# HpWang-whu/RoReg

Hardware: AMD Instinct MI355X
Metric: pair-registrations/sec (higher is better)
Workload: dtype f32 (every f32 operand enters the fp16 matrix cores as hi + lo fp16 under a per-keypoint power-of-two block scale: <= 22 significant bits relative to a CONSERVATIVE per-keypoint bound -- measured on the extractor: the bound sits 2^2..2^6 above the keypoint's true coefficient maximum (config.f16x2_sc

## Files before the change

include/roreg_hip.h:

```cpp
#ifndef ROREG_HIP_H
#define ROREG_HIP_H

#include <stdint.h>
#include <stddef.h>

#ifdef __cplusplus
extern "C" {
#endif

#define ROREG_ABI_VERSION 6
int roreg_abi_version(void);
const char *roreg_last_error(void);

int roreg_set_group_tables(const int32_t *P_host, const int32_t *Nei_host, const double *R_host);

size_t roreg_group_conv_packed_size(int Cin, int Cout, int KS);
int roreg_group_conv_pack_weights(const float *W_host , int Cin, int Cout, int KS,
                                  float *wpack_host );
size_t roreg_group_conv_workspace_size(int B, int Cin, int Cout, int Lin, int Lout, int KS);
int roreg_group_conv(const float *x, const float *wpack, const float *bias,
                     const float *bn_scale, const float *bn_shift, const float *residual,
                     float *out, const int32_t *gather,
                     int B, int Cin, int Cout, int Lin, int Lout, int KS,
                     float *workspace, size_t workspace_floats, void *stream);
// ... 215 lines not shown
size_t roreg_irrep_gemm_tiles(int O, int B, int32_t *tiles_host);
size_t roreg_irrep_gemm_tiles_m(int O, int B, int tile_m , int32_t *tiles_host);
int roreg_irrep_gemm(const float *const *X, float *const *Out, const float *const *Add, const float *const *Wpack, int C, int O, int B,
                     const int32_t *tiles_dev, int n_tiles, void *stream);
int roreg_irrep_gemm_split(const float *const *X, float *const *Out, const float *const *Add, const void *const *Wsplit, int C, int O, int B,
                           const int32_t *tiles_dev, int n_tiles, void *stream);
int roreg_irrep_gemm_f16x2(const float *const *X, float *const *Out, const float *const *Add, const void *const *Wsplit2,
                           const float *x_bound_dev, int w_exp, const float *next_u_dev, const float *next_v_dev, float *out_bound_dev,
                           int C, int O, int B, const int32_t *tiles_dev, int n_tiles,
                           int tile_m ,
                           int x_planes , void *stream);
int roreg_gemm_persistent(int on);
int roreg_gemm_thin(int on);
int roreg_irrep_gemm_f16x2_rows(const float *const *X, float *T3r, const void *const *Wsplit2, const float *x_bound_dev, int w_exp, int C, int B, void *stream);
int roreg_gf_finish(const float *T3r, const float *x, const float *b_out, const float *role_scale , const float *role_shift ,
                    float *eqv, float *inv, float *role_out , float *eqv_ft, int B, void *stream);
int roreg_gf_finish_route(int on);
int roreg_row_bound(const void *x_spatial, int x_bf16 , const float *bn_scale, const float *bn_shift,
                    float *bound_out, int B, int C, void *stream);
int roreg_ft_nonlin(const float *Xin , const float *x_spatial, const float *bias,
                    const float *bias2, const float *bn_scale, const float *bn_shift, const float *resid_spatial,
                    float *Xout , float *out_spatial ,
                    const int32_t *g_map ,
                    int Lout , int Lvalid,
                    int B, int C, int split ,
                    const float *out_bound ,
                    float *out_rowmax ,
                    int spatial_bf16 ,
                    int out_planes ,
                    void *stream);
int roreg_ft_nonlin_packed(const float *Xin, const float *bias, const float *bn_scale, const float *bn_shift, uint32_t *out_words,
                           const int32_t *g_map, int Lout, int Lvalid, int B, int C, const float *out_bound, float *raw_col, int raw_g,
                           void *stream);
int roreg_ft_nonlin_gathered(const uint64_t *rows , const int64_t *dr , int feat_bf16, const float *bn_scale ,
                             const float *bn_shift, float *Xout, int B, const float *out_bound , int out_planes, void *stream);

typedef struct roreg_icp_grid_desc {
    double origin[3];
    double edge;
    int32_t dims[3];
    int32_t n;
    int64_t cells;
    int64_t reserved;
} roreg_icp_grid_desc;
size_t roreg_icp_grid_size(const double *lo_host, const double *hi_host, int n, double max_dist, roreg_icp_grid_desc *desc_host,
                           size_t *workspace_bytes);
int roreg_icp_grid_build(const float *points, const roreg_icp_grid_desc *desc_host, void *grid, void *workspace, size_t workspace_bytes,
                         void *stream);
typedef struct roreg_icp_task {
    const void *tgt_grid;
    const void *src_grid;
    const double *T0;
    int32_t n_src;
    int32_t slot0;
} roreg_icp_task;
size_t roreg_icp_batch_workspace(int n_tasks, long long total_slots);
int roreg_icp_batch(const roreg_icp_task *tasks, int n_tasks, const int32_t *work, int n_work, long long total_slots, double max_dist,
                    int max_iter, double tol_deg, double tol_t, double *T_out, int32_t *iters_out, int32_t *inliers_out, double *rmse_out,
                    int32_t *status_out, int32_t *assign_out, double *stats_out, void *workspace, size_t workspace_bytes, void *stream);

int roreg_icp_normals(const void *grid, double radius, int min_neighbors, double *out, void *stream);
typedef struct roreg_icp_plane_task {
    const void *tgt_grid;
    const void *src_grid;
    const double *tgt_normals;
    const double *T0;
// ... 151 lines not shown
```

roreg_amd/_abi.py:

```python
import ctypes
from ctypes import c_int, c_void_p, c_size_t, c_double, c_float, c_char_p

import numpy as np

ABI_VERSION = 6

_P = c_void_p
PROTOTYPES = {
    'roreg_abi_version': (c_int, []),
    'roreg_last_error': (c_char_p, []),
    'roreg_set_group_tables': (c_int, [_P, _P, _P]),
    'roreg_group_conv_packed_size': (c_size_t, [c_int, c_int, c_int]),
    'roreg_group_conv_pack_weights': (c_int, [_P, c_int, c_int, c_int, _P]),
    'roreg_group_conv_workspace_size': (c_size_t, [c_int, c_int, c_int, c_int, c_int, c_int]),
    'roreg_group_conv': (c_int, [_P, _P, _P, _P, _P, _P, _P, _P, c_int, c_int, c_int, c_int, c_int, c_int, _P, c_size_t, _P]),
    'roreg_group_conv_split': (c_int, [_P, _P, _P, _P, _P, _P, _P, _P, c_int, c_int, c_int, c_int, c_int, c_int, c_int, _P]),
    'roreg_group_conv_f16x2': (c_int, [_P, _P, c_int, _P, _P, _P, c_float, c_float, _P, _P, _P, _P, _P, c_int, c_int, c_int, c_int, c_int, c_int, c_int, _P]),
    'roreg_group_conv_f16x2_packed': (c_int, [_P, _P, c_int, _P, _P, _P, _P, _P, _P, c_int, c_int, c_int, c_int, c_int, c_int, c_int, _P]),
    'roreg_dense_f16x2': (c_int, [_P, _P, c_int, _P, _P, _P, c_float, c_float, _P, _P, c_int, _P, _P, c_int, c_int, c_int, _P]),
    'roreg_dense_split': (c_int, [_P, _P, _P, _P, _P, _P, c_int, _P, c_int, c_int, c_int, _P]),
    'roreg_gf_finalize': (c_int, [_P, _P, c_int, _P, c_int, _P]),
    'roreg_det_score': (c_int, [_P, _P, c_int, _P]),
    'roreg_inv_descriptor': (c_int, [_P, c_int, _P, c_int, _P]),
    'roreg_nn_search': (c_int, [_P, _P, c_int, _P, _P, c_int, c_int, _P, _P, _P, _P]),
# ... 24 lines not shown
    'roreg_row_bound_roles': (c_int, [_P, c_int, _P, _P, _P, _P, c_int, _P]),
    'roreg_inv_descriptor_roles': (c_int, [_P, c_int, _P, _P, _P, _P, c_int, _P]),
    'roreg_lt_prepare_rows': (c_int, [_P, _P, c_int, c_int, c_int, _P, _P, _P, _P]),
    'roreg_ransac_batch_workspace': (c_size_t, [c_int, ctypes.c_longlong, c_int]),
    'roreg_ransac_batch': (c_int, [_P, c_int, ctypes.c_longlong, c_int, c_int, c_double, c_int, _P, _P, _P, _P, _P, _P, c_size_t, _P]),
    'roreg_refine_batch': (c_int, [_P, _P, c_int, ctypes.c_longlong, _P, ctypes.c_double, c_int, _P, _P, _P, _P]),
    'roreg_yohoc_draw': (c_int, [_P, ctypes.c_longlong, _P, _P, c_int, c_int, _P, _P, _P, _P]),
    'roreg_gather_rows_batch': (c_int, [_P, c_int, c_int, c_int, _P]),
    'roreg_gather_rows_f64': (c_int, [_P, _P, c_int, c_int, _P, _P]),
    'roreg_group_corr': (c_int, [_P, _P, _P, _P, c_int, c_int, _P, _P, _P]),
    'roreg_topk_dot_workspace_size': (c_size_t, [c_int, c_int, c_int]),
    'roreg_topk_dot': (c_int, [_P, c_int, _P, c_int, c_int, _P, _P, _P, c_size_t, _P, _P, c_int, c_int, c_int, _P]),
    'roreg_context_colmax': (c_int, [_P, c_int, _P, c_int, c_int, _P, _P, _P]),
    'roreg_sinkhorn_batch_workspace_size': (c_size_t, [c_int, c_int, c_int, ctypes.c_longlong, ctypes.c_longlong]),
    'roreg_sinkhorn_batch_consts': (c_int, [_P, _P, c_int, _P]),
    'roreg_sinkhorn_batch': (c_int, [_P, _P, _P, _P, _P, _P, _P, c_int, c_float, c_int, _P, _P, _P, _P, _P, c_size_t, _P]),
    'roreg_sinkhorn_batch2_workspace_size': (c_size_t, [c_int, c_int, c_int, ctypes.c_longlong, ctypes.c_longlong]),
    'roreg_sinkhorn_batch2': (c_int, [_P, _P, _P, _P, _P, _P, _P, c_int, c_float, c_int, _P, _P, _P, _P, _P, c_size_t, c_int, _P]),
    'roreg_sinkhorn_batch3_workspace_size': (c_size_t, [c_int, c_int, c_int, ctypes.c_longlong, ctypes.c_longlong, c_int, c_int]),
    'roreg_sinkhorn_batch3': (c_int, [_P, _P, _P, _P, _P, _P, _P, c_int, c_float, c_int, _P, _P, _P, _P, _P, c_size_t, c_int, _P, _P]),
    'roreg_write_files': (c_int, [_P, _P, _P, _P, _P, c_int, c_int]),
    'roreg_yohoc_draw_many': (c_int, [_P, c_int, _P, _P, c_int, c_int, _P, _P, _P, c_int]),
    'roreg_mlp_head_workspace': (c_size_t, [c_int, c_int, c_int]),
    'roreg_mlp_head': (c_int, [_P, _P, _P, _P, _P, c_int, c_int, c_int, c_int, _P, _P, c_int, _P, _P, _P, _P, _P, c_int, c_int, c_float, _P, _P, _P]),
    'roreg_sinkhorn_early_exit': (c_int, [c_int]),
    'roreg_sinkhorn_iteration_stats': (c_int, [_P, _P, c_int, _P]),
    'roreg_linear': (c_int, [_P, c_int, c_int, _P, _P, c_int, _P, _P]),
    'roreg_linear_mfma': (c_int, [_P, c_int, c_int, _P, _P, c_int, _P, _P]),
    'roreg_linear_path': (c_int, [c_int]),
    'roreg_linear_cat3': (c_int, [_P, _P, _P, _P, c_int, c_int, _P, _P, c_int, _P, _P]),
    'roreg_gemm_persistent': (c_int, [c_int]),
    'roreg_gemm_thin': (c_int, [c_int]),
    'roreg_gf_finish_route': (c_int, [c_int]),
    'roreg_irrep_gemm_f16x2_rows': (c_int, [_P, _P, _P, _P, c_int, c_int, c_int, _P]),
    'roreg_gf_finish': (c_int, [_P, _P, _P, _P, _P, _P, _P, _P, _P, c_int, _P]),
    'roreg_instnorm_stats': (c_int, [_P, c_int, c_int, c_float, _P, _P, _P, c_int, c_int, _P]),
    'roreg_mlp_tail': (c_int, [_P, c_int, c_int, _P, _P, _P, _P, _P, c_int, c_int, _P]),
    'roreg_mlp_tail_mfma': (c_int, [_P, c_int, c_int, _P, _P, _P, _P, _P, c_int, c_int, _P]),
    'roreg_knn_attention': (c_int, [_P, _P, _P, _P, c_int, c_int, c_int, c_int, _P, _P]),
    'roreg_rm_elementwise': (c_int, [c_int, _P, _P, _P, _P, c_int, c_int, c_int, _P, _P, _P]),
    'roreg_sinkhorn_workspace_size': (c_size_t, [c_int, c_int]),
    'roreg_sinkhorn': (c_int, [_P, c_int, _P, c_int, c_float, c_int, _P, _P, _P, _P, _P, _P, c_size_t, _P]),
    'roreg_icp_grid_size': (c_size_t, [_P, _P, c_int, c_double, _P, _P]),
    'roreg_icp_grid_build': (c_int, [_P, _P, _P, _P, c_size_t, _P]),
    'roreg_icp_batch_workspace': (c_size_t, [c_int, ctypes.c_longlong]),
    'roreg_icp_batch': (c_int, [_P, c_int, _P, c_int, ctypes.c_longlong, c_double, c_int, c_double, c_double, _P, _P, _P, _P, _P, _P, _P, _P, c_size_t, _P]),
    'roreg_icp_normals': (c_int, [_P, c_double, c_int, _P, _P]),
    'roreg_icp_plane_batch_workspace': (c_size_t, [c_int, ctypes.c_longlong]),
    'roreg_icp_plane_batch': (c_int, [_P, c_int, _P, c_int, ctypes.c_longlong, c_double, c_int, c_double, c_double, _P, _P, _P, _P, _P, _P, _P, _P, c_size_t, _P]),
    'roreg_icp_gicp_batch_workspace': (c_size_t, [c_int, ctypes.c_longlong]),
    'roreg_icp_gicp_batch': (c_int, [_P, c_int, _P, c_int, ctypes.c_longlong, c_double, c_int, c_double, c_double, _P, _P, _P, _P, _P, _P, _P, _P, c_size_t, _P]),
    'roreg_icp_plane_robust_batch_workspace': (c_size_t, [c_int, ctypes.c_longlong]),
    'roreg_icp_plane_robust_batch': (c_int, [_P, c_int, _P, c_int, ctypes.c_longlong, c_double, c_int, c_double, c_double, _P, _P, _P, _P, _P, _P, _P, _P, c_size_t, _P]),
    'roreg_icp_gicp_robust_batch_workspace': (c_size_t, [c_int, ctypes.c_longlong]),
    'roreg_icp_gicp_robust_batch': (c_int, [_P, c_int, _P, c_int, ctypes.c_longlong, c_double, c_int, c_double, c_double, _P, _P, _P, _P, _P, _P, _P, _P, c_size_t, _P]),
    'roreg_icp_eval_workspace': (c_size_t, [c_int, ctypes.c_longlong]),
    'roreg_icp_eval_batch': (c_int, [_P, c_int, _P, c_int, ctypes.c_longlong, c_double, _P, _P, _P, _P, _P, c_size_t, _P]),
    'roreg_voxel_workspace': (c_size_t, [c_int]),
    'roreg_voxel_downsample': (c_int, [_P, c_int, c_double, _P, _P, _P, _P, _P, _P, _P, c_size_t, _P]),
    'roreg_pg_workspace': (c_size_t, [_P, c_int]),
    'roreg_pg_optimize_batch': (c_int, [_P, _P, c_int, _P, _P, _P, _P, _P, _P, _P, _P, _P, _P, _P, c_int, c_int, _P, _P, _P, _P, _P, _P, _P, _P, _P, _P, _P, c_size_t, _P]),
    'roreg_sparse_map_workspace': (c_size_t, [c_int]),
    'roreg_sparse_stride_map': (c_int, [_P, c_int, c_int, _P, c_int, _P, _P, _P, _P, _P, c_size_t, _P]),
    'roreg_sparse_kernel_map': (c_int, [_P, c_int, _P, c_int, c_int, c_int, _P, _P, _P, c_size_t, _P]),
    'roreg_sparse_conv': (c_int, [_P, c_int, c_int, c_int, _P, c_int, c_int, _P, c_int, _P, _P, _P, c_int, c_int, _P, c_int, _P]),
    'roreg_sparse_l2norm': (c_int, [_P, c_int, c_int, _P, _P]),
# ... 66 lines not shown
```

roreg_amd/_hip_fourier.py:

```python
import os
from ctypes import c_void_p

import numpy as np
import torch

from . import hip as _core
from .hip import HipError, _check, _feat, _ptr, _stream, lib

__all__ = ['DenseSplitLayer', 'IRREP_DIMS', 'IRREP_OFFSETS', '_bf16_split3', '_keypoint_of_columns', '_ptr_array', '_res_ptr', '_tile_cache', 'bf16_split3_frags', 'bf16_split3_pack', 'bound_exp', 'coef_pitch', 'coef_size', 'coef_views', 'dense_split', 'ensure_fourier', 'f16_scale_exp', 'f16_split2_frags', 'f16_split2_pack', 'frag_pack', 'ft_nonlin', 'ft_nonlin_gathered', 'ft_nonlin_packed', 'gemm_persistent', 'gemm_thin', 'gf_finish', 'gf_finish_rows', 'gf_finish_usable', 'group_conv_split_pack', 'irrep_gemm', 'irrep_gemm_rows', 'next_bound', 'next_bound_spatial', 'pack_coefs_f16x2', 'row_bound', 'unpack_coefs_f16x2', 'words_to_planes']


_fourier_ready = False
IRREP_DIMS = (1, 3, 3, 4, 5)
IRREP_OFFSETS = (0, 1, 10, 19, 35, 60)


def ensure_fourier():
    global _fourier_ready
    if not _fourier_ready:
        from .fourier import group_fourier
        F = np.ascontiguousarray(group_fourier().F, np.float32)
        _check(lib().roreg_set_fourier_tables(F.ctypes.data), 'roreg_set_fourier_tables')
        _fourier_ready = True


def _ptr_array(views):
    arr = (c_void_p * 5)(*[c_void_p(v.data_ptr()) for v in views])
    return arr


def coef_pitch(B):
    return (int(B) + 31) // 32 * 32


def coef_size(C, B):
    return 60 * C * coef_pitch(B)


def coef_views(buf, C, B):
    Bp = coef_pitch(B)
    return [buf[IRREP_OFFSETS[r] * C * Bp:IRREP_OFFSETS[r + 1] * C * Bp].view(IRREP_DIMS[r] * C, IRREP_DIMS[r] * Bp) for r in range(5)]

# ... 50 lines not shown
    if _core.PROFILE is not None:
        e1.record(); _core.PROFILE.append((('irrep_gemm_f16x2' if f16x2 is not None else 'irrep_gemm_split' if split is not None else 'irrep_gemm', Bp, C, O), e0, e1))
    return (out, bound_out) if next_bound is not None else out


class _GemmSwitch:

    def __init__(self, entry, coerce, doc, on=None):
        self.entry, self.coerce, self.__doc__, self.on = entry, coerce, doc, on

    def __call__(self, on=True):
        return _GemmSwitch(self.entry, self.coerce, self.__doc__, self.coerce(on))

    def __enter__(self):
        self.prev = getattr(lib(), self.entry)(self.on)

    def __exit__(self, *exc):
        getattr(lib(), self.entry)(self.prev)
        return False


gemm_persistent = _GemmSwitch('roreg_gemm_persistent', int,
                              """`with hip.gemm_persistent(True | False):` -- how the 16x16x32 LDS-DMA GEMM is launched inside the block (roreg_gemm_persistent): persistent
    workgroups that claim tiles, or one workgroup per tile.  Same bits either way -- tests and A/B measurements.""")
gemm_thin = _GemmSwitch('roreg_gemm_thin', lambda on: int(bool(on)),
                        """`with hip.gemm_thin(True | False):` -- whether the thin layers (C == 32 or O == 32, fp16 x 2, word layout, no residual) run on their own
    kernels inside the block (roreg_gemm_thin; the default) or on the generic one.  Same bits either way -- tests and A/B measurements.""")

gf_finish = _GemmSwitch('roreg_gf_finish_route', lambda on: int(bool(on)),
                        """`with hip.gf_finish(True | False):` -- whether the engine ends the extractor with Conv_out in per-keypoint rows + gf_finish_kernel (roreg_gf_finish_route;
    the default, ROREG_GF_FINISH=0 in the environment turns it off) or with the four kernels ft_nonlin, gf_finalize, inv_descriptor, feat_coefs.  Same bits either
    way -- tests and A/B measurements.""")


def gf_finish_usable(gemm_mode, *dtypes):
    return (gemm_mode == 'f16x2' and _core.GEMM_MODE == 'f16x2' and all(d == torch.float32 for d in dtypes)
            and lib().roreg_gemm_thin(-1) == 1 and lib().roreg_gf_finish_route(-1) == 1)


def irrep_gemm_rows(X_buf, C, B, f16x2, x_bound):
    Bp = coef_pitch(B)
    wl, w_exp = f16x2
    if X_buf.numel() != 60 * C * Bp or x_bound is None or x_bound.numel() != Bp:
        raise HipError(f'irrep_gemm_rows: X_buf must hold 60*C*{Bp} words and x_bound {Bp} values')
    out = torch.empty((Bp, 60, 32), dtype=torch.float32, device=X_buf.device)
    _check(lib().roreg_irrep_gemm_f16x2_rows(_ptr_array(coef_views(X_buf, C, B)), _ptr(out), _ptr_array(wl), _ptr(x_bound, torch.float32), int(w_exp), C, Bp,
                                             _stream()), 'roreg_irrep_gemm_f16x2_rows')
    return out


def gf_finish_rows(T3r, x, b_out, roles=None):
    ensure_fourier()
    B = int(x.shape[0])
    if x.shape[1:] != (32, 60) or x.dtype != torch.float32 or not x.is_contiguous() or T3r.shape != (coef_pitch(B), 60, 32) or b_out.numel() != 32:
        raise HipError('gf_finish_rows: T3r [Bp,60,32], x [B,32,60] contiguous float32, b_out [32]')
    eqv = torch.empty((B, 32, 60), dtype=torch.float32, device=x.device)
    eft = torch.empty((B, 32, 60), dtype=torch.float32, device=x.device)
    inv = torch.empty((B, 32), dtype=torch.float32, device=x.device)
    scale = shift = role = None
    if roles is not None:
        scale, shift, role = _core._role_args(roles, B)
        scale, shift = scale[64:], shift[64:]
    _check(lib().roreg_gf_finish(_ptr(T3r, torch.float32), _ptr(x, torch.float32), _ptr(b_out, torch.float32), _ptr(scale), _ptr(shift), _ptr(eqv), _ptr(inv),
                                 _ptr(role), _ptr(eft), B, _stream()), 'roreg_gf_finish')
    return eqv, inv, eft

# ... 43 lines not shown
        o.copy_(w.view(torch.float32))
    return out, bound


def words_to_planes(X_words, C, B):
    w = X_words.contiguous().view(torch.int32).view(-1, 2, 16)
    hi = (w & 0xffff).to(torch.int16).transpose(1, 2); lo = (w >> 16).to(torch.int16).transpose(1, 2)
    return torch.cat([hi.reshape(-1, 32), lo.reshape(-1, 32)], 1).contiguous().view(torch.float32).view(-1)


def unpack_coefs_f16x2(X_words, bound, C, B):
    Bp = coef_pitch(B)
    e = bound_exp(bound)
    out = torch.empty_like(X_words)
    for r, (v, o) in enumerate(zip(coef_views(X_words, C, B), coef_views(out, C, B))):
        kp = _keypoint_of_columns(IRREP_DIMS[r], Bp)
        w = v.view(torch.int32)
        hi = (w & 0xffff).to(torch.int16).view(torch.float16).float()
        lo = (w >> 16).to(torch.int16).view(torch.float16).float()
        o.copy_(torch.ldexp(hi + lo, -e[kp][None, :]))
    return out


def next_bound_spatial(bn, bias):
    scale, shift = bn
    sc = scale.detach().double().abs().cpu(); sh = shift.detach().double().abs().cpu()
    b = bias.detach().double().cpu()
    k = 1.0 + 2.0 ** -9
    u = (np.sqrt(60.0) * k) * sc
    v = k * (sc * b.abs() + sh) + 1e-30
    return u.float().cuda().contiguous(), v.float().cuda().contiguous()


def ft_nonlin_packed(B, C, coef_in, bias, bn, out_bound, g_map=None, Lout=60, Lvalid=60, raw_g=None):
    ensure_fourier()
    dev = coef_in.device
    if coef_in.numel() != coef_size(C, B) or out_bound.numel() != coef_pitch(B):
        raise HipError('ft_nonlin_packed: coef_in / out_bound sizes')
    words = torch.empty((B, C, Lout if g_map is not None else 60), dtype=torch.int32, device=dev)
    raw = torch.empty((B, C), dtype=torch.float32, device=dev) if raw_g is not None else None
    scale, shift = bn if bn is not None else (None, None)
    _check(lib().roreg_ft_nonlin_packed(_ptr(coef_in, torch.float32), _ptr(bias), _ptr(scale), _ptr(shift), _ptr(words), _ptr(g_map, torch.int32),
                                        int(Lout), int(Lvalid), B, C, _ptr(out_bound, torch.float32), _ptr(raw), int(raw_g or 0), _stream()),
           'roreg_ft_nonlin_packed')
    return words, raw


def next_bound(bn, bias, bias2=None):
    scale, shift = bn
    sc = scale.detach().double().abs().cpu(); sh = shift.detach().double().abs().cpu()
    b = bias.detach().double().cpu() + (bias2.detach().double().cpu() if bias2 is not None else 0.0)
    k = 1.0 + 2.0 ** -9
    u = (60.0 * k) * sc
    v = (np.sqrt(60.0) * k) * (sc * b.abs() + sh) + 1e-30
    return u.float().cuda().contiguous(), v.float().cuda().contiguous()


def ft_nonlin(B, C, coef_in=None, x_spatial=None, bias=None, bias2=None, bn=None, resid_spatial=None, spatial_out=False,
              g_map=None, Lout=60, Lvalid=60, split=False, out_bound=None, want_rowmax=False, planes=False):
    ensure_fourier()
    dev = (coef_in if coef_in is not None else x_spatial).device
    if spatial_out:
        out = torch.empty((B, C, Lout if g_map is not None else 60), dtype=torch.float32, device=dev); xout = None; osp = _ptr(out)
    else:
        out = torch.empty(coef_size(C, B), dtype=torch.float32, device=dev); xout = _ptr(out); osp = None
    scale, shift = bn if bn is not None else (None, None)
    if want_rowmax and not spatial_out:
        raise HipError('ft_nonlin: want_rowmax goes with spatial_out')
    amax = torch.zeros(B, dtype=torch.float32, device=dev) if want_rowmax else None
    if coef_in is not None and coef_in.numel() != coef_size(C, B):
        raise HipError(f'ft_nonlin: coef_in must hold 60*C*{coef_pitch(B)} floats')
    if out_bound is not None and out_bound.numel() != coef_pitch(B):
        raise HipError(f'ft_nonlin: out_bound must hold one value per (padded) keypoint ({coef_pitch(B)})')
# ... 119 lines not shown
```

roreg_amd/csrc/fourier.hip:

```cpp
#include "common.h"
#include "primitives.h"
#include <algorithm>
#include <atomic>
#include <cmath>
#include <cstdlib>
#include <type_traits>
#include <utility>
#include <vector>

namespace {

constexpr int NIRR = 5;

struct GemmDescs {
    const float *X[NIRR];
    float *Out[NIRR];
    const float *Add[NIRR];
    const float4 *W[NIRR];
    int K[NIRR], M[NIRR], Mpad[NIRR], N[NIRR];
};

__device__ __forceinline__ void lds_dma16(const void *src, void *dst) {
    __builtin_amdgcn_global_load_lds((const __attribute__((address_space(1))) void *)src, (__attribute__((address_space(3))) void *)dst, 16, 0, 0);
}
// ... 1984 lines not shown
                    unsigned *dst = reinterpret_cast<unsigned *>(const_cast<char *>(slot_ptr(ic, p.Xout, c, tb)));
                    if (kPS.kind[S] != 2 || h == 0) __builtin_nontemporal_store(word, dst);
                });
            } else {
                const int tb = tbi;
                static_for<32>([&](auto ic) {
                    constexpr int S = decltype(ic)::value, t = S / 16, r = S % 16;
                    float *dst = reinterpret_cast<float *>(const_cast<char *>(slot_ptr(ic, p.Xout, c, tb)));
                    if (kPS.kind[S] != 2 || h == 0) __builtin_nontemporal_store(o[t][r], dst);
                });
            }
        }
    };
    if (wave_global < n_tiles) {
        const int last = wave_global + ((n_tiles - 1 - wave_global) / n_waves) * n_waves;
        float cb[NCV + 1];
        GDesc da{0u, 0u, 0}, db{0u, 0u, 0};
        if constexpr (GATHER) {
            da = load_desc(wave_global);
            db = load_desc(min(wave_global + n_waves, last));
            load_rows_gathered(wave_global, da, cn);
        } else {
            load_coefs(wave_global, cn);
        }
        __builtin_amdgcn_s_waitcnt(0x0F70);
        for (int tile = wave_global; tile <= last; tile += 2 * n_waves) {
            const int t1 = min(tile + n_waves, last), t2 = min(tile + 2 * n_waves, last), t3 = min(tile + 3 * n_waves, last);
            process(tile, t1, cn, cb, t2, db, da);
            process(t1, t2, cb, cn, t3, da, db);
        }
    }
}

#undef OFF_OF
#undef OFF_Q

struct GfFinishParams {
    const float *T3r;
    const float *x;
    const float *b_out;
    const float *role_scale, *role_shift;
    float *eqv, *inv, *role_out, *eqv_ft;
    const f16x8 *A1h, *A2h;
    int f_exp, B;
};

__global__ __launch_bounds__(256, 2) void gf_finish_kernel(GfFinishParams p) {
    constexpr int NA = 4 * 2 * 2 * 64 * 4;
    extern __shared__ __attribute__((aligned(16))) float gf_smem[];
    float *sA1 = gf_smem, *sA2 = gf_smem + NA, *sT = gf_smem + 2 * NA, *sRole = sT + 4 * 32 * 65;
    const int lane = threadIdx.x & 63, jn = lane & 31, h = lane >> 5;
    {
        const float *g1 = reinterpret_cast<const float *>(p.A1h), *g2 = reinterpret_cast<const float *>(p.A2h);
        for (int i = threadIdx.x; i < NA; i += 256) { sA1[i] = g1[i]; sA2[i] = g2[i]; }
        if (threadIdx.x < 128) sRole[threadIdx.x] = p.role_scale ? (threadIdx.x < 64 ? p.role_scale[threadIdx.x] : p.role_shift[threadIdx.x - 64]) : 0.f;
    }
    __syncthreads();
    const f16x8 *sA1h = reinterpret_cast<const f16x8 *>(sA1), *sA2h = reinterpret_cast<const f16x8 *>(sA2);
    const int wave_global = __builtin_amdgcn_readfirstlane((blockIdx.x * 256 + threadIdx.x) >> 6);
    const int n_waves = gridDim.x * 4;
    const int B = p.B;
    const bool act = lane < ROREG_G;
    const float bo = p.b_out[jn] + 0.f;
    float *ti = sT + (threadIdx.x >> 6) * (32 * 65);

    auto load = [&](int b, float (&cv)[32], float (&xv)[32]) {
// ... 330 lines not shown
        p.X[r] = X[r]; p.Out[r] = Out[r]; p.Add[r] = Add ? Add[r] : nullptr; p.W[r] = reinterpret_cast<const float4 *>(Wpack[r]);
        p.K[r] = dims[r] * C; p.M[r] = dims[r] * O; p.Mpad[r] = round_up(dims[r] * O, 128); p.N[r] = dims[r] * B;
    }
    constexpr int CT = 32;
    const size_t lds = 2 * CT * 256 * sizeof(float);
    return roreg::launch_lds("roreg_irrep_gemm", irrep_gemm_kernel<CT>, dim3(n_tiles), dim3(256), lds, roreg::as_stream(stream), p, tiles_dev);
}

struct GemmSwitch {
    const char *env;
    int dflt, hi;
    std::atomic<int> v{-1};
    int get() {
        int x = v.load(std::memory_order_relaxed);
        if (x < 0) {
            const char *e = getenv(env);
            x = e && e[0] >= '0' && e[0] <= '0' + hi ? e[0] - '0' : dflt;
            v.store(x, std::memory_order_relaxed);
        }
        return x;
    }
    int set(int on) {
        const int prev = get();
        if (on >= 0 && on <= hi) v.store(on, std::memory_order_relaxed);
        return prev;
    }
};
static GemmSwitch g_gemm_persist{"ROREG_GEMM_PERSIST", 0, 2};
static GemmSwitch g_gf_finish{"ROREG_GF_FINISH", 1, 1};
static GemmSwitch g_gemm_thin{"ROREG_GEMM_THIN", 1, 1};
extern "C" int roreg_gemm_persistent(int on) { return g_gemm_persist.set(on); }
extern "C" int roreg_gemm_thin(int on) { return g_gemm_thin.set(on); }
extern "C" int roreg_gf_finish_route(int on) { return g_gf_finish.set(on); }
static int gemm_cu_count() {
    static const int n = [] {
        int dev = 0, cus = 0;
        if (hipGetDevice(&dev) != hipSuccess || hipDeviceGetAttribute(&cus, hipDeviceAttributeMultiprocessorCount, dev) != hipSuccess || cus <= 0) cus = 256;
        return cus;
    }();
    return n;
}
template <int NP, int WO>
static int launch_gemm_split(const char *what, const float *const *X, float *const *Out, const float *const *Add, const void *const *Wsplit,
                             const float *xbound, int w_exp, const float *nb_u, const float *nb_v, float *out_bound, int C, int O, int B,
                             const int32_t *tiles_dev, int n_tiles, void *stream, int x_planes = 0) {
    static const int dims[5] = {1, 3, 3, 4, 5};
    GemmSplitDescs p;
    for (int r = 0; r < 5; ++r) {
        p.X[r] = X[r]; p.Out[r] = Out[r]; p.Add[r] = Add ? Add[r] : nullptr; p.W[r] = Wsplit[r];
        p.K[r] = dims[r] * C; p.M[r] = dims[r] * O; p.Mpad[r] = round_up(dims[r] * O, 128); p.N[r] = dims[r] * B;
        if (WO == 4 && p.Mpad[r] % 256 != 0) { roreg::set_error("%s: tile_m = 256 needs O %% 256 == 0 (got %d)", what, O); return 2; }
    }
    p.out_rows = 0;
    p.xbound = xbound; p.w_exp = w_exp; p.nb_u = nb_u; p.nb_v = nb_v; p.out_bound = out_bound; p.O = O;
    if constexpr (NP == 2) {
        if (!x_planes && !Add && (O == 32 || (C == 32 && O % 32 == 0 && O <= 512)) && g_gemm_thin.get()) {
            int wgs = 0;
            for (int r = 0; r < 5; ++r) { const int tc = C == 32 ? thin_tile_cols<false>(r) : thin_tile_cols<true>(r); wgs += (p.N[r] + tc - 1) / tc; }
            if (C == 32) hipLaunchKernelGGL(irrep_gemm_thin_k_kernel, dim3(wgs), dim3(512), 0, roreg::as_stream(stream), p);
            else hipLaunchKernelGGL(irrep_gemm_thin_m_kernel, dim3(wgs), dim3(256), 0, roreg::as_stream(stream), p);
            hipError_t e2 = hipGetLastError();
            if (e2 != hipSuccess) { roreg::set_error("%s: launch failed: %s", what, hipGetErrorString(e2)); return 1; }
            return 0;
        }
    }
    auto launch = [&](auto kern, int wgs, int threads, size_t lds, auto... more) {
// ... 162 lines not shown
        else launch_ft<ft_nonlin_kernel<false, true, 2, 4, 1>>(p, n_tiles, s);
    } else if (split == 1) {
        if (in_sp) launch_ft<ft_nonlin_kernel<true, false, 3, 4, 1>>(p, n_tiles, s);
        else if (!out_sp) launch_ft<ft_nonlin_kernel<false, false, 3, 4, 1>>(p, n_tiles, s);
        else launch_ft<ft_nonlin_kernel<false, true, 3, 4, 1>>(p, n_tiles, s);
    } else {
        if (in_sp) launch_ft<ft_nonlin_kernel<true, false, 0, 4, 1>>(p, n_tiles, s);
        else if (!out_sp) launch_ft<ft_nonlin_kernel<false, false, 0, 4, 1>>(p, n_tiles, s);
        else launch_ft<ft_nonlin_kernel<false, true, 0, 4, 1>>(p, n_tiles, s);
    }
    ROREG_CHECK_LAUNCH("roreg_ft_nonlin");
    return 0;
}

extern "C" int roreg_ft_nonlin_packed(const float *Xin, const float *bias, const float *bn_scale, const float *bn_shift, uint32_t *out_words,
                                      const int32_t *g_map, int Lout, int Lvalid, int B, int C, const float *out_bound, float *raw_col, int raw_g,
                                      void *stream) {
    ROREG_REQUIRE(g_A1 && g_A2, "roreg_ft_nonlin_packed: roreg_set_fourier_tables has not been called");
    ROREG_REQUIRE(Xin && out_words && out_bound && B > 0 && C > 0 && C <= 512 && (bn_scale == nullptr) == (bn_shift == nullptr), "roreg_ft_nonlin_packed: bad arguments");
    ROREG_REQUIRE(!g_map || (Lout >= Lvalid && Lvalid > 0 && Lout <= 64), "roreg_ft_nonlin_packed: bad Lout/Lvalid");
    ROREG_REQUIRE(!raw_col || (raw_g >= 0 && raw_g < ROREG_G), "roreg_ft_nonlin_packed: raw_g out of range");
    NonlinParams p;
    memset(&p, 0, sizeof(p));
    p.Xin = Xin; p.out_spatial = reinterpret_cast<float *>(out_words);
    p.g_map = g_map; p.Lout = g_map ? Lout : ROREG_G; p.Lvalid = g_map ? Lvalid : ROREG_G;
    p.bias = bias; p.bn_scale = bn_scale; p.bn_shift = bn_shift; p.A1 = g_A1; p.A2 = g_A2;
    p.A1s = reinterpret_cast<const bf16x8 *>(g_A1s); p.A2s = reinterpret_cast<const bf16x8 *>(g_A2s);
    p.A1h = reinterpret_cast<const f16x8 *>(g_A1h); p.A2h = reinterpret_cast<const f16x8 *>(g_A2h); p.f_exp = g_f_exp;
    p.out_bound = out_bound; p.sp_pack = 1; p.raw_col = raw_col; p.raw_g = raw_g;
    p.B = B; p.Bp = (B + 31) / 32 * 32; p.C = C; p.tiles_per_c = (B + 31) / 32;
    ROREG_REQUIRE((unsigned long long)C * p.Bp * 20ull < (1ull << 32), "roreg_ft_nonlin_packed: C * round_up(B, 32) must stay below 2^32 / 20 (32-bit lane offsets)");
    hipStream_t s = roreg::as_stream(stream);
    roreg::ProfScope prof(roreg::PROF_FT_NONLIN, s);
    launch_ft<ft_nonlin_kernel<false, true, 2, 4, 1>>(p, (long long)C * p.tiles_per_c, s);
    ROREG_CHECK_LAUNCH("roreg_ft_nonlin_packed");
    return 0;
}

extern "C" int roreg_ft_nonlin_gathered(const uint64_t *rows, const int64_t *dr, int feat_bf16, const float *bn_scale, const float *bn_shift, float *Xout,
                                        int B, const float *out_bound, int out_planes, void *stream) {
    ROREG_REQUIRE(g_A1 && g_A2, "roreg_ft_nonlin_gathered: roreg_set_fourier_tables has not been called");
    ROREG_REQUIRE(roreg::group_tables().ready, "roreg_ft_nonlin_gathered: group tables not set");
    ROREG_REQUIRE(rows && dr && Xout && out_bound && B > 0 && (bn_scale == nullptr) == (bn_shift == nullptr), "roreg_ft_nonlin_gathered: bad arguments");
    constexpr int C = 4 * ROREG_F;
    ROREG_REQUIRE((long long)60 * C * B < (1ll << 40), "roreg_ft_nonlin_gathered: tensor too large");
    NonlinParams p;
    memset(&p, 0, sizeof(p));
    p.Xout = Xout; p.Lout = ROREG_G; p.Lvalid = ROREG_G;
    p.bn_scale = bn_scale; p.bn_shift = bn_shift; p.A1 = g_A1; p.A2 = g_A2;
    p.A1s = reinterpret_cast<const bf16x8 *>(g_A1s); p.A2s = reinterpret_cast<const bf16x8 *>(g_A2s);
    p.A1h = reinterpret_cast<const f16x8 *>(g_A1h); p.A2h = reinterpret_cast<const f16x8 *>(g_A2h); p.f_exp = g_f_exp;
    p.out_bound = out_bound; p.x_bf16 = feat_bf16; p.out_planes = out_planes;
    p.g_rows = reinterpret_cast<const roreg::LtRow *>(rows); p.g_dr = dr; p.g_P8 = roreg::group_tables().P8;
    p.B = B; p.Bp = (B + 31) / 32 * 32; p.C = C; p.tiles_per_c = (B + 31) / 32;
    ROREG_REQUIRE((unsigned long long)C * p.Bp * 20ull < (1ull << 32), "roreg_ft_nonlin_gathered: 128 * round_up(B, 32) must stay below 2^32 / 20 (32-bit lane offsets)");
    hipStream_t s = roreg::as_stream(stream);
    roreg::ProfScope prof(roreg::PROF_FT_NONLIN, s);
    launch_ft<ft_nonlin_kernel<true, false, 2, 4, 1, false, true>>(p, (long long)C * p.tiles_per_c, s);
    ROREG_CHECK_LAUNCH("roreg_ft_nonlin_gathered");
    return 0;
}

extern "C" int roreg_feat_coefs(const void *x, int x_bf16, float *out, int B, int C, int split, void *stream) {
    if (B == 0) return 0;
    ROREG_REQUIRE(g_A1 && g_A2, "roreg_feat_coefs: roreg_set_fourier_tables has not been called");
    ROREG_REQUIRE(x && out && B > 0 && C > 0 && C <= 512 && split >= 0 && split <= 2, "roreg_feat_coefs: bad arguments");
// ... 54 lines not shown
```

Before: 1132.

## Add persistent LDS-staged inverse-transform pack kernel for ft_nonlin_packed

Measured after the change: 1142, median of 6. About the same (+0.9%).

```diff
diff --git a/include/roreg_hip.h b/include/roreg_hip.h
--- a/include/roreg_hip.h
+++ b/include/roreg_hip.h
@@ -271,6 +271,7 @@
 int roreg_ft_nonlin_packed(const float *Xin, const float *bias, const float *bn_scale, const float *bn_shift, uint32_t *out_words,
                            const int32_t *g_map, int Lout, int Lvalid, int B, int C, const float *out_bound, float *raw_col, int raw_g,
                            void *stream);
+int roreg_ift_packed_route(int on);
 int roreg_ft_nonlin_gathered(const uint64_t *rows , const int64_t *dr , int feat_bf16, const float *bn_scale ,
                              const float *bn_shift, float *Xout, int B, const float *out_bound , int out_planes, void *stream);
 
diff --git a/roreg_amd/_abi.py b/roreg_amd/_abi.py
--- a/roreg_amd/_abi.py
+++ b/roreg_amd/_abi.py
@@ -80,6 +80,7 @@
     'roreg_gemm_persistent': (c_int, [c_int]),
     'roreg_gemm_thin': (c_int, [c_int]),
     'roreg_gf_finish_route': (c_int, [c_int]),
+    'roreg_ift_packed_route': (c_int, [c_int]),
     'roreg_irrep_gemm_f16x2_rows': (c_int, [_P, _P, _P, _P, c_int, c_int, c_int, _P]),
     'roreg_gf_finish': (c_int, [_P, _P, _P, _P, _P, _P, _P, _P, _P, c_int, _P]),
     'roreg_instnorm_stats': (c_int, [_P, c_int, c_int, c_float, _P, _P, _P, c_int, c_int, _P]),
diff --git a/roreg_amd/_hip_fourier.py b/roreg_amd/_hip_fourier.py
--- a/roreg_amd/_hip_fourier.py
+++ b/roreg_amd/_hip_fourier.py
@@ -7,7 +7,7 @@
 from . import hip as _core
 from .hip import HipError, _check, _feat, _ptr, _stream, lib
 
-__all__ = ['DenseSplitLayer', 'IRREP_DIMS', 'IRREP_OFFSETS', '_bf16_split3', '_keypoint_of_columns', '_ptr_array', '_res_ptr', '_tile_cache', 'bf16_split3_frags', 'bf16_split3_pack', 'bound_exp', 'coef_pitch', 'coef_size', 'coef_views', 'dense_split', 'ensure_fourier', 'f16_scale_exp', 'f16_split2_frags', 'f16_split2_pack', 'frag_pack', 'ft_nonlin', 'ft_nonlin_gathered', 'ft_nonlin_packed', 'gemm_persistent', 'gemm_thin', 'gf_finish', 'gf_finish_rows', 'gf_finish_usable', 'group_conv_split_pack', 'irrep_gemm', 'irrep_gemm_rows', 'next_bound', 'next_bound_spatial', 'pack_coefs_f16x2', 'row_bound', 'unpack_coefs_f16x2', 'words_to_planes']
+__all__ = ['DenseSplitLayer', 'IRREP_DIMS', 'IRREP_OFFSETS', '_bf16_split3', '_keypoint_of_columns', '_ptr_array', '_res_ptr', '_tile_cache', 'bf16_split3_frags', 'bf16_split3_pack', 'bound_exp', 'coef_pitch', 'coef_size', 'coef_views', 'dense_split', 'ensure_fourier', 'f16_scale_exp', 'f16_split2_frags', 'f16_split2_pack', 'frag_pack', 'ft_nonlin', 'ft_nonlin_gathered', 'ft_nonlin_packed', 'gemm_persistent', 'gemm_thin', 'gf_finish', 'gf_finish_rows', 'gf_finish_usable', 'group_conv_split_pack', 'ift_packed', 'irrep_gemm', 'irrep_gemm_rows', 'next_bound', 'next_bound_spatial', 'pack_coefs_f16x2', 'row_bound', 'unpack_coefs_f16x2', 'words_to_planes']
 
 
 _fourier_ready = False
@@ -124,6 +124,11 @@
     the default, ROREG_GF_FINISH=0 in the environment turns it off) or with the four kernels ft_nonlin, gf_finalize, inv_descriptor, feat_coefs.  Same bits either
     way -- tests and A/B measurements.""")
 
+ift_packed = _GemmSwitch('roreg_ift_packed_route', lambda on: int(bool(on)),
+                         """`with hip.ift_packed(True | False):` -- whether ft_nonlin_packed runs ift_pack_kernel where it applies (roreg_ift_packed_route; the default,
+    ROREG_IFT_PACKED=0 in the environment turns it off) or the transform kernel's own instantiation everywhere.  Same bits either way -- tests and A/B
+    measurements.""")
+
 
 def gf_finish_usable(gemm_mode, *dtypes):
     return (gemm_mode == 'f16x2' and _core.GEMM_MODE == 'f16x2' and all(d == torch.float32 for d in dtypes)
@@ -233,13 +238,20 @@
     return u.float().cuda().contiguous(), v.float().cuda().contiguous()
 
 
-def ft_nonlin_packed(B, C, coef_in, bias, bn, out_bound, g_map=None, Lout=60, Lvalid=60, raw_g=None):
+def ft_nonlin_packed(B, C, coef_in, bias, bn, out_bound, g_map=None, Lout=60, Lvalid=60, raw_g=None, out=None):
     ensure_fourier()
     dev = coef_in.device
     if coef_in.numel() != coef_size(C, B) or out_bound.numel() != coef_pitch(B):
         raise HipError('ft_nonlin_packed: coef_in / out_bound sizes')
-    words = torch.empty((B, C, Lout if g_map is not None else 60), dtype=torch.int32, device=dev)
-    raw = torch.empty((B, C), dtype=torch.float32, device=dev) if raw_g is not None else None
+    wshape = (B, C, Lout if g_map is not None else 60)
+    if out is not None:
+        words, raw = out
+        if (words.shape != wshape or words.dtype != torch.int32 or not words.is_contiguous() or (raw is None) != (raw_g is None)
+                or (raw is not None and (raw.shape != (B, C) or raw.dtype != torch.float32 or not raw.is_contiguous()))):
+            raise HipError('ft_nonlin_packed: out = (int32 [B,C,Lout], float32 [B,C] or None), contiguous')
+    else:
+        words = torch.empty(wshape, dtype=torch.int32, device=dev)
+        raw = torch.empty((B, C), dtype=torch.float32, device=dev) if raw_g is not None else None
     scale, shift = bn if bn is not None else (None, None)
     _check(lib().roreg_ft_nonlin_packed(_ptr(coef_in, torch.float32), _ptr(bias), _ptr(scale), _ptr(shift), _ptr(words), _ptr(g_map, torch.int32),
                                         int(Lout), int(Lvalid), B, C, _ptr(out_bound, torch.float32), _ptr(raw), int(raw_g or 0), _stream()),
diff --git a/roreg_amd/csrc/fourier.hip b/roreg_amd/csrc/fourier.hip
--- a/roreg_amd/csrc/fourier.hip
+++ b/roreg_amd/csrc/fourier.hip
@@ -2040,6 +2040,159 @@
     }
 }
 
+__host__ __device__ constexpr int ift_pack_pitch(int Lout) { return (4 * Lout + 8) % 8 == 4 ? 4 * Lout + 8 : 4 * Lout + 12; }
+constexpr int IFT_NA1 = 4 * 2 * 2 * 64 * 4;
+__host__ __device__ constexpr size_t ift_pack_lds_bytes(int Lout, int C) { return sizeof(float) * ((size_t)2 * 32 * ift_pack_pitch(Lout) + IFT_NA1 + 3 * (size_t)C + 64); }
+
+__global__ __launch_bounds__(256, 2) void ift_pack_kernel(NonlinParams p) {
+    typedef unsigned u32x4 __attribute__((ext_vector_type(4)));
+    extern __shared__ __attribute__((aligned(16))) float ip_smem[];
+    const int lane = threadIdx.x & 63, jn = lane & 31, h = lane >> 5;
+    const int w = __builtin_amdgcn_readfirstlane((int)threadIdx.x >> 6);
+    const int B = p.B, C = p.C, Lout = p.Lout;
+    const int P = ift_pack_pitch(Lout), img_words = 32 * P;
+    unsigned *img = reinterpret_cast<unsigned *>(ip_smem);
+    float *sA1 = ip_smem + 2 * img_words;
+    float *sBias = sA1 + IFT_NA1, *sScale = sBias + C, *sShift = sScale + C;
+    int *sGmap = reinterpret_cast<int *>(sShift + C);
+    {
+        if (threadIdx.x < 64) sGmap[threadIdx.x] = threadIdx.x < ROREG_G ? (p.g_map ? p.g_map[threadIdx.x] : (int)threadIdx.x) : -1;
+        const float *g1 = reinterpret_cast<const float *>(p.A1h);
+        for (int i = threadIdx.x; i < IFT_NA1; i += 256) sA1[i] = g1[i];
+        for (int i = threadIdx.x; i < 2 * img_words; i += 256) img[i] = 0u;
+        for (int i = threadIdx.x; i < C; i += 256) {
+            sBias[i] = (p.bias ? p.bias[i] : 0.f) + 0.f;
+            sScale[i] = p.bn_scale ? p.bn_scale[i] : 1.f;
+            sShift[i] = p.bn_shift ? p.bn_shift[i] : 0.f;
+        }
+    }
+    __syncthreads();
+    const int key = jn >> 3;
+    unsigned woff[32];
+    static_for<32>([&](auto ic) {
+        constexpr int t = decltype(ic)::value / 16, r = decltype(ic)::value % 16;
+        const int g = t * 32 + (r & 3) + 8 * (r >> 2) + 4 * h;
+        const int go = sGmap[g];
+        const int col = (go >= 0 && go < p.Lvalid) ? w * Lout + go : 4 * Lout + 4;
+        woff[t * 16 + r] = (unsigned)(jn * P + (col ^ key)) * 4u;
+    });
+    const bool has_raw = p.raw_col != nullptr;
+    const int raw_slot = (p.raw_g >> 5) * 16 + (p.raw_g & 3) + 4 * ((p.raw_g & 31) >> 3);
+    const bool raw_mine = has_raw && ((p.raw_g >> 2) & 1) == h;
+    const unsigned raw_off = (unsigned)(jn * P + ((raw_mine ? 4 * Lout + w : 4 * Lout + 4) ^ key)) * 4u;
+    const int n_act = Lout + (has_raw ? 1 : 0);
+    const int lr = lane < n_act ? lane : n_act - 1;
+    char *const st_base = lr < Lout ? reinterpret_cast<char *>(p.out_spatial) + 16 * lr : reinterpret_cast<char *>(p.raw_col);
+    const unsigned st_unit = lr < Lout ? 4u * (unsigned)Lout : 4u;
+    const f16x8 *sA1h = reinterpret_cast<const f16x8 *>(sA1);
+    const size_t Bp = (size_t)p.Bp;
+    const size_t hmask = (size_t)0 - (size_t)h;
+    const int tpc = p.tiles_per_c;
+    auto load_coefs = [&](int u, float (&dst)[33]) {
+        const int cg = u / tpc, tb = u - cg * tpc, c = 4 * cg + w;
+        dst[32] = p.out_bound[tb * 32 + jn];
+        static_for<32>([&](auto ic) {
+            constexpr int st = decltype(ic)::value / 8, e = decltype(ic)::value % 8;
+            constexpr int q0 = 16 * st + e, q1 = 16 * st + 8 + e;
+            if constexpr (q1 < ROREG_G) dst[st * 8 + e] = __builtin_nontemporal_load(p.Xin + OFF_OF(q0, q1, c, tb) + jn);
+            else dst[st * 8 + e] = __builtin_nontemporal_load(p.Xin + OFF_Q(q0, c, tb) + jn);
+        });
+    };
+    auto table_mma = [&](const f16x8 *a, const f16x8 (&b)[2], f32x16 c) {
+        f16x8 av[2];
+#pragma unroll
+        for (int pl = 0; pl < 2; ++pl) av[pl] = a[64 * pl];
+        return split_mma<2>(av, b, c);
+    };
+    auto column_scale = [&](float mx, float &xscale, float &oscale) {
+        mx = fmaxf(mx, __shfl_xor(mx, 32));
+        int e = 0;
+        if (mx > 0.f && mx < __builtin_inff()) { int ex; (void)frexpf(mx, &ex); e = 14 - ex; }
+        xscale = ldexpf(1.f, e); oscale = ldexpf(1.f, -(e + p.f_exp));
+    };
+    auto process = [&](int u, int next_u, float (&cv)[33], float (&cnext)[33], unsigned *im) {
+        asm volatile("" ::: "memory");
+        const int cg = u / tpc, tbi = u - cg * tpc, c0 = 4 * cg, c = c0 + w;
+        const bool valid = tbi * 32 + jn < B;
+        load_coefs(next_u, cnext);
+        __builtin_amdgcn_sched_barrier(0);
+        f32x16 v[2];
+#pragma unroll
+        for (int t = 0; t < 2; ++t)
+#pragma unroll
+            for (int r = 0; r < 16; ++r) v[t][r] = 0.f;
+        {
+            float mx = 0.f;
+#pragma unroll
+            for (int s = 0; s < 32; ++s) mx = fmaxf(mx, ((16 * (s >> 3) + 8 + (s & 7) < ROREG_G || h == 0) ? fabsf(cv[s]) : 0.f));
+            float xsc, osc;
+            column_scale(mx, xsc, osc);
+#pragma unroll
+            for (int st = 0; st < 4; ++st) {
+                float x8[8];
+#pragma unroll
+                for (int e = 0; e < 8; ++e) x8[e] = (16 * st + 8 + e < ROREG_G || h == 0) ? cv[st * 8 + e] : 0.f;
+                f16x8 bh, bl;
+                split2(x8, xsc, bh, bl);
+                const f16x8 b[2] = {bh, bl};
+                v[0] = table_mma(sA1h + ((st * 2 + 0) * 2) * 64 + lane, b, v[0]);
+                v[1] = table_mma(sA1h + ((st * 2 + 1) * 2) * 64 + lane, b, v[1]);
+            }
+#pragma unroll
+            for (int t = 0; t < 2; ++t)
+#pragma unroll
+                for (int r = 0; r < 16; ++r) v[t][r] *= osc;
+        }
+        const float bsum = sBias[c], sc = sScale[c], sh = sShift[c];
+        const float pk_scale = ldexpf(1.f, bound_exp(cv[32]));
+        char *const imb = reinterpret_cast<char *>(im);
+        auto epilogue = [&](auto bnc) {
+            float xraw = 0.f;
+#pragma unroll
+            for (int t = 0; t < 2; ++t)
+#pragma unroll
+                for (int r = 0; r < 16; ++r) {
+                    const int g = t * 32 + (r & 3) + 8 * (r >> 2) + 4 * h;
+                    float x = v[t][r] + bsum;
+                    if (t * 16 + r == raw_slot) xraw = x;
+                    if constexpr (decltype(bnc)::value) x = fmaxf(fmaf(x, sc, sh), 0.f);
+                    if (g >= ROREG_G || !valid) x = 0.f;
+                    const float xs = x * pk_scale;
+                    const _Float16 h1 = (_Float16)xs;
+                    const _Float16 l1 = (_Float16)(xs - (float)h1);
+                    *reinterpret_cast<unsigned *>(imb + woff[t * 16 + r]) =
+                        (unsigned)__builtin_bit_cast(unsigned short, h1) | ((unsigned)__builtin_bit_cast(unsigned short, l1) << 16);
+                }
+            *reinterpret_cast<float *>(imb + raw_off) = xraw;
+        };
+        if (p.bn_scale) epilogue(std::true_type{}); else epilogue(std::false_type{});
+        asm volatile("s_waitcnt lgkmcnt(0)\n\ts_barrier" ::: "memory");
+        const unsigned row0 = (unsigned)(tbi * 32) * (unsigned)C + (unsigned)c0;
+        const int kp_last = min(32, B - tbi * 32) - 1;
+        u32x4 q[8];
+#pragma unroll
+        for (int i = 0; i < 8; ++i) q[i] = *reinterpret_cast<const u32x4 *>(imb + (min(4 * i + w, kp_last) * P + 4 * lr) * 4);
+#pragma unroll
+        for (int i = 0; i < 8; ++i) {
+            const int kp = min(4 * i + w, kp_last);
+            const bool k0 = (kp >> 3) & 1, k1 = (kp >> 4) & 1;
+            const u32x4 a = k0 ? u32x4{q[i][1], q[i][0], q[i][3], q[i][2]} : q[i];
+            const u32x4 o = k1 ? u32x4{a[2], a[3], a[0], a[1]} : a;
+            *reinterpret_cast<u32x4 *>(st_base + (size_t)(row0 + (unsigned)kp * (unsigned)C) * st_unit) = o;
+        }
+    };
+    const int n_units = (C >> 2) * tpc;
+    const int u0 = (int)((long long)blockIdx.x * n_units / gridDim.x), last = (int)((long long)(blockIdx.x + 1) * n_units / gridDim.x) - 1;
+    float cn[33], cb[33];
+    load_coefs(u0, cn);
+    __builtin_amdgcn_s_waitcnt(0x0F70);
+    for (int u = u0; u <= last; u += 2) {
+        const int t1 = min(u + 1, last), t2 = min(u + 2, last);
+        process(u, t1, cn, cb, img);
+        process(t1, t2, cb, cn, img + img_words);
+    }
+}
+
 #undef OFF_OF
 #undef OFF_Q
 
@@ -2436,6 +2589,8 @@
 extern "C" int roreg_gemm_persistent(int on) { return g_gemm_persist.set(on); }
 extern "C" int roreg_gemm_thin(int on) { return g_gemm_thin.set(on); }
 extern "C" int roreg_gf_finish_route(int on) { return g_gf_finish.set(on); }
+static GemmSwitch g_ift_packed{"ROREG_IFT_PACKED", 1, 1};
+extern "C" int roreg_ift_packed_route(int on) { return g_ift_packed.set(on); }
 static int gemm_cu_count() {
     static const int n = [] {
         int dev = 0, cus = 0;
@@ -2664,6 +2819,13 @@
     ROREG_REQUIRE((unsigned long long)C * p.Bp * 20ull < (1ull << 32), "roreg_ft_nonlin_packed: C * round_up(B, 32) must stay below 2^32 / 20 (32-bit lane offsets)");
     hipStream_t s = roreg::as_stream(stream);
     roreg::ProfScope prof(roreg::PROF_FT_NONLIN, s);
+    const bool aligned = (reinterpret_cast<uintptr_t>(out_words) | reinterpret_cast<uintptr_t>(raw_col)) % 16 == 0;
+    if (g_ift_packed.get() && C % 4 == 0 && aligned && p.Lout + (raw_col ? 1 : 0) <= 64) {
+        const size_t lds = ift_pack_lds_bytes(p.Lout, C);
+        static const int rounds = [] { const char *e = getenv("ROREG_FT_ROUNDS"); const int r = e ? atoi(e) : 0; return r > 0 ? r : 4; }();
+        const long long want = (long long)(C / 4) * p.tiles_per_c, cap = (long long)(2 * lds <= 160 * 1024 ? 2 : 1) * gemm_cu_count() * rounds;
+        return roreg::launch_lds("roreg_ft_nonlin_packed", ift_pack_kernel, dim3((unsigned)(want > cap ? cap : want)), dim3(256), lds, s, p);
+    }
     launch_ft<ft_nonlin_kernel<false, true, 2, 4, 1>>(p, (long long)C * p.tiles_per_c, s);
     ROREG_CHECK_LAUNCH("roreg_ft_nonlin_packed");
     return 0;
```
